# kluonj/HelFEM

Measured on AMD Instinct MI355X. Metric: scf_iteration_wall_time_fock_plus_geneig_nbf4230, lower is better.
Workload: dtype f64; 1 GPU; diatomic Z1=7 Z2=7 R=2.068 PBE, nelem=5 nnodes=15 nquad=75 lmmax=[20,20] (Nbf=4230, Nang=61, Nrad=70), XC grid 92x13, symmetry blocks [1380, 1470, 1380]: J+XC Fock build + eig_gsym_sub + density per step; parallelism=shard1, density=occupied orbitals of the core Hamiltonian

## Files before the change

### helfem_amd/csrc/hip/capi.cpp

```cpp
#include "internal.h"
#include "../host/checkpoint.h"
#include "../host/diis.h"
#include "../host/dftfuncs.h"
#include <cstring>
#include <memory>
#include <mutex>

namespace hfg {
static thread_local std::string g_err;
void set_error(const std::string &msg) { g_err = msg; }

}

using namespace hfg;

#define HFG_TRY try {
#define HFG_CATCH                       \
  }                                     \
  catch (const std::logic_error &e) {   \
    hfg::set_error(e.what());           \
    return 1;                           \
  }                                     \
  catch (const std::runtime_error &e) { \
    hfg::set_error(e.what());           \
// ... 664 lines not shown
  if (nP == 0) return false;
  if (!in || !out) throw std::logic_error(std::string(who) + ": null matrix pointer\n");
  return true;
}
int hfg_coulomb_batch_devptr(hfg_ctx *ctx, hfg_basis *b, int64_t nP, const double *dP, double *dJ) {
  HFG_TRY
  if (coulomb_batch_args("hfg_coulomb_batch_devptr", ctx, b, nP, dP, dJ)) coulomb_batch_dev(ctx, b, nP, dP, dJ);
  HFG_CATCH
}
int hfg_exchange_dev(hfg_ctx *ctx, hfg_basis *b, const double *dP, double *dK) {
  HFG_TRY exchange_dev(ctx, b, dP, dK);
  HFG_CATCH
}
int hfg_exchange_occ_dev(hfg_ctx *ctx, hfg_basis *b, const double *dP, const double *dC, int64_t nocc, double *dK) {
  HFG_TRY
  if (nocc < 1 || !dC) throw std::logic_error("hfg_exchange_occ_dev: occupied orbitals missing\n");
  exchange_dev(ctx, b, dP, dK, false, dC, (int)nocc);
  HFG_CATCH
}
int hfg_rs_exchange_dev(hfg_ctx *ctx, hfg_basis *b, const double *dP, double *dK) {
  HFG_TRY exchange_dev(ctx, b, dP, dK, true);
  HFG_CATCH
}
int hfg_xc_fock_dev(hfg_ctx *ctx, hfg_basis *b, int x_func, int c_func, const double *dP, double *dH, double *dScal,
                    double thr) {
  HFG_TRY xc_fock_dev(ctx, b, x_func, c_func, dP, dH, dScal, thr);
  HFG_CATCH
}
int hfg_xc_fock_pol_dev(hfg_ctx *ctx, hfg_basis *b, int x_func, int c_func, const double *dPa, const double *dPb,
                        double *dHa, double *dHb, double *dScal, double thr) {
  HFG_TRY xc_fock_pol_dev(ctx, b, x_func, c_func, dPa, dPb, dHa, dHb, dScal, thr);
  HFG_CATCH
}
int hfg_eig_gsym_sub_dev(hfg_ctx *ctx, int64_t N, const double *dF, const double *dS, int nblk, const int64_t *blk_ptr,
                         const int64_t *blk_idx, double *dE, double *dC) {
  HFG_TRY eig_gsym_sub_dev(ctx, (int)N, dF, dS, nblk, blk_ptr, blk_idx, dE, dC);
  HFG_CATCH
}
int64_t hfg_eig_block_buf_size(int nblk, const int64_t *blk_ptr) { return (int64_t)eig_block_buf_size(nblk, blk_ptr); }
int hfg_eig_blocks_dev(hfg_ctx *ctx, int64_t N, const double *dF, const double *dS, int nblk, const int64_t *blk_ptr,
                       const int64_t *blk_idx, double *dBlockBuf) {
  HFG_TRY eig_blocks_dev(ctx, (int)N, dF, dS, nblk, blk_ptr, blk_idx, dBlockBuf);
  HFG_CATCH
}
int hfg_eig_assemble_dev(hfg_ctx *ctx, int64_t N, int nblk, const int64_t *blk_ptr, const int64_t *blk_idx,
                         const double *dBlockBuf, double *dE, double *dC) {
  HFG_TRY eig_assemble_dev(ctx, (int)N, nblk, blk_ptr, blk_idx, dBlockBuf, dE, dC);
  HFG_CATCH
}
int hfg_form_density_dev(hfg_ctx *ctx, int64_t N, int64_t ncols, const double *dC, int64_t nocc, double *dP) {
  HFG_TRY form_density_dev(ctx, (int)N, (int)ncols, dC, (int)nocc, dP);
  HFG_CATCH
}
int hfg_gemm_dev(hfg_ctx *ctx, int tA, int tB, int64_t m, int64_t n, int64_t k, const double *dA, int64_t lda,
                 const double *dB, int64_t ldb, double *dC, int64_t ldc) {
  HFG_TRY gemm_dev(ctx, tA != 0, tB != 0, (int)m, (int)n, (int)k, 1.0, dA, (int)lda, dB, (int)ldb, 0.0, dC, (int)ldc);
  HFG_CATCH
}

int64_t hfg_fock_compact_size(hfg_basis *b) { return (int64_t)fock_compact_size(b); }
int hfg_fock_compact_dev(hfg_ctx *ctx, hfg_basis *b, int x_func, int c_func, const double *dP, double *dFc,
                         double *dScal, double thr) {
  HFG_TRY fock_compact_dev(ctx, b, x_func, c_func, dP, dFc, dScal, thr);
  HFG_CATCH
}
int hfg_fock_finish_dev(hfg_ctx *ctx, hfg_basis *b, const double *dFc, const double *dH0, const int *dBlockId,
// ... 410 lines not shown
```

### helfem_amd/csrc/hip/fock.hip

```cpp
#include "internal.h"
#include "xc_device.h"
#include "../host/dftfuncs.h"
#include <cstring>

namespace hfg {

__global__ void k_gather_compact(const double *__restrict__ P, int N, int A, int R, int E, int p,
                                 const int *__restrict__ shell_off, const int *__restrict__ shell_skip,
                                 double *__restrict__ Xc) {
  int blk = blockIdx.x;
  int e = blk % E;
  int xy = blk / E;
  int y = xy % A, x = xy / A;
  int pp = p * p;
  for (int t = threadIdx.x; t < pp; t += blockDim.x) {
    int i = t % p, j = t / p;
    int ni = e * (p - 1) + i, nj = e * (p - 1) + j;
    double v = 0.0;
    bool ok = (ni < R) && (nj < R) && !(shell_skip[x] && ni == 0) && !(shell_skip[y] && nj == 0);
    if (ok) v = P[(size_t)(shell_off[y] + nj) * N + (shell_off[x] + ni)];
    Xc[(size_t)blk * pp + t] = v;
  }
}

// ... 524 lines not shown
          s0 += sB[i * nq + q] * pv;
          s1 += sdB[i * nq + q] * pv;
        }
        d0 += s0 * sB[j * nq + q];
        d1 += s1 * sB[j * nq + q];
        d2 += s1 * sdB[j * nq + q];
        if (do_lapl) d3 += s0 * sL[j * nq + q];
      }
    if (q < nq && jc < NJ) {
      part[(0 * NJ + jc) * nq + q] = d0;
      part[(1 * NJ + jc) * nq + q] = d1;
      part[(2 * NJ + jc) * nq + q] = d2;
      if (do_lapl) part[(3 * NJ + jc) * nq + q] = d3;
    }
    __syncthreads();
    if (jc == 0 && q < nq && (e * nq + q) % nranks == rank) {
      double a0 = 0.0, a1 = 0.0, a2 = 0.0, a3 = 0.0;
      for (int k = 0; k < NJ; k++) {
        a0 += part[(0 * NJ + k) * nq + q];
        a1 += part[(1 * NJ + k) * nq + q];
        a2 += part[(2 * NJ + k) * nq + q];
        if (do_lapl) a3 += part[(3 * NJ + k) * nq + q];
      }
      const size_t Q = (size_t)e * nq + q;
      D0[Q * AA + xy] = a0;
      if (do_grad) D1[Q * AA + xy] = a1;
      if (do_tau) D2[Q * AA + xy] = a2;
      if (do_lapl) D3[Q * AA + xy] = a3;
    }
    __syncthreads();
  }
}

__global__ void k_xc_density_theta(const double *__restrict__ D0, const double *__restrict__ D1,
                                   const double *__restrict__ D2, const double *__restrict__ D3, const double *__restrict__ Th,
                                   const double *__restrict__ dTh, const int *__restrict__ shell_l,
                                   const double *__restrict__ rad_sh, int A, int nth, int G,
                                   const int *__restrict__ grp_off, const int *__restrict__ grp_shell, int do_grad,
                                   int do_tau, int do_lapl, size_t NQ, int rank, int nranks, double *__restrict__ V) {
  extern __shared__ double sh[];
  size_t Q = blockIdx.x;
  if ((int)(Q % nranks) != rank) return;
  int ga = blockIdx.y / G, gb = blockIdx.y % G;
  int a0 = grp_off[ga], na = grp_off[ga + 1] - a0;
  int b0 = grp_off[gb], nb = grp_off[gb + 1] - b0;
  double *d0 = sh, *d1 = sh + na * nb, *d2 = sh + 2 * na * nb, *d3 = sh + 3 * na * nb;
  size_t AA = (size_t)A * A;
  const double ir2 = do_lapl ? 1.0 / (rad_sh[Q] * rad_sh[Q]) : 0.0;
  for (int t = threadIdx.x; t < na * nb; t += blockDim.x) {
    int ia = t / nb, ib = t % nb;
    int a = grp_shell[a0 + ia], b = grp_shell[b0 + ib];
    d0[t] = D0[Q * AA + (size_t)a * A + b];
    d1[t] = do_grad ? D1[Q * AA + (size_t)a * A + b] : 0.0;
    d2[t] = do_tau ? D2[Q * AA + (size_t)a * A + b] : 0.0;
    if (do_lapl) d3[t] = D3[Q * AA + (size_t)a * A + b] - (double)(shell_l[b] * (shell_l[b] + 1)) * ir2 * d0[t];
  }
  __syncthreads();
  for (int i = threadIdx.x; i < nth; i += blockDim.x) {
    double r = 0.0, s = 0.0, u = 0.0, k3 = 0.0, k4 = 0.0, k5 = 0.0;
    for (int ia = 0; ia < na; ia++) {
      int a = grp_shell[a0 + ia];
      double s0 = 0.0, s1 = 0.0, s2 = 0.0, s3 = 0.0, s5 = 0.0;
      for (int ib = 0; ib < nb; ib++) {
        double tb = Th[(size_t)grp_shell[b0 + ib] * nth + i];
        s0 += d0[ia * nb + ib] * tb;
        s1 += d1[ia * nb + ib] * tb;
// ... 915 lines not shown
  XCPlan pl;
  pl.do_grad = either(xc::is_gga);
  pl.do_lapl = either(xc::is_mgga_lapl);
  if (pl.do_lapl && t->geom != 1) throw std::logic_error("Laplacian not implemented!\n");
  pl.do_tau = either(xc::is_mgga) || pl.do_lapl;
  pl.ext = either(xc::is_ext);
  pl.thr = pl.do_tau ? std::max(thr, 1e-40) : thr;
  pl.maxgrp = 0;
  for (int g = 0; g < t->G; g++) pl.maxgrp = std::max(pl.maxgrp, t->h_grp_off[g + 1] - t->h_grp_off[g]);
  pl.NQ = (size_t)t->E * t->nq;
  pl.AA = (size_t)t->A * t->A;
  pl.nv = pl.NQ * t->G * t->G * t->ntheta;
  return pl;
}

static void xc_buffers(FockAux &a, const XCPlan &pl, int planes) {
  a.D0.resize(pl.NQ * pl.AA);
  a.D1.resize(pl.NQ * pl.AA);
  a.GA.resize(pl.NQ * pl.AA);
  a.GB.resize(pl.NQ * pl.AA);
  if (pl.do_tau) {
    a.D2.resize(pl.NQ * pl.AA);
    a.GC.resize(pl.NQ * pl.AA);
  }
  if (pl.do_lapl) {
    a.D3.resize(pl.NQ * pl.AA);
    a.GL.resize(pl.NQ * pl.AA);
  }
  a.V.resize(planes * pl.nv);
  a.Fo.resize(planes * pl.nv);
  a.partial.resize(3 * pl.NQ);
}

static void xc_density_stage(hfg_ctx *ctx, const hfg_dev_tables *t, FockAux &a, const XCPlan &pl, const double *dPc, double *dV) {
  const int A = t->A, E = t->E, p = t->p, nq = t->nq, G = t->G, nth = t->ntheta;
  hipLaunchKernelGGL(k_xc_density_radial, dim3(A * A, E), dim3(256), xc_density_radial_lds(p, nq, pl.do_lapl), ctx->stream, dPc,
                     t->rad_B.p, t->rad_dB.p, (const double *)t->rad_L.p, A, E, p, nq, pl.do_grad, pl.do_tau, pl.do_lapl,
                     ctx->shard_rank, ctx->shard_n, a.D0.p, a.D1.p, a.D2.p, a.D3.p);
  hipLaunchKernelGGL(k_xc_density_theta, dim3((unsigned)pl.NQ, G * G), dim3(std::min(256, round_up64(nth))),
                     (pl.do_lapl ? 4 : 3) * pl.maxgrp * pl.maxgrp * sizeof(double), ctx->stream, a.D0.p, a.D1.p, (const double *)a.D2.p,
                     (const double *)a.D3.p, t->Th.p, t->dTh.p, t->shell_l.p, t->rad_sh.p, A, nth, G, t->grp_off.p, t->grp_shell.p,
                     pl.do_grad, pl.do_tau, pl.do_lapl, pl.NQ, ctx->shard_rank, ctx->shard_n, dV);
}

static void xc_fock_stage(hfg_ctx *ctx, const hfg_dev_tables *t, FockAux &a, const XCPlan &pl, double *dFo, double *dHc) {
  const int A = t->A, E = t->E, p = t->p, nq = t->nq;
  launch_xc_fock_theta(ctx, pl.NQ, t->G, t->ntheta, pl.maxgrp, dFo, t->Th.p, t->dTh.p, A, t->grp_off.p, t->grp_shell.p, pl.do_grad,
                       pl.do_tau, ctx->shard_rank, ctx->shard_n, a.GA.p, a.GB.p, a.GC.p, pl.do_lapl, a.GL.p);
  hipLaunchKernelGGL(k_xc_fock_radial, dim3(A * A, E), dim3(std::min(256, round_up64(p * p))), xc_fock_radial_lds(p, nq, pl.do_lapl),
                     ctx->stream, a.GA.p, a.GB.p, (const double *)a.GC.p, (const double *)a.GL.p, t->rad_B.p, t->rad_dB.p,
                     (const double *)t->rad_L.p, t->shell_l.p, t->rad_sh.p, A, E, p, nq, pl.do_grad, pl.do_tau, pl.do_lapl, ctx->shard_rank,
                     ctx->shard_n, dHc);
}

template <typename K, typename... Tail>
static void launch_xc_grid(hfg_ctx *ctx, const hfg_dev_tables *t, FockAux &a, const XCPlan &pl, K k_ext, K k_plain, size_t shb,
                           int x_func, int c_func, Tail... tail) {
  K k = pl.ext ? k_ext : k_plain;
  if (shb > 64 * 1024) HFG_HIP_CHECK(hipFuncSetAttribute((const void *)k, hipFuncAttributeMaxDynamicSharedMemorySize, (int)shb));
  hipLaunchKernelGGL(k, dim3((unsigned)pl.NQ), dim3(256), shb, ctx->stream, a.V.p, t->rad_w.p, t->rad_sh.p, t->th_s.p, t->th_w.p,
                     t->grp_m.p, t->cosd.p, t->sind.p, t->Dmax, t->G, t->ntheta, t->nphi, t->Rhalf, t->geom, x_func, c_func, pl.do_grad,
                     pl.do_tau, pl.do_lapl, pl.thr, pl.NQ, ctx->shard_rank, ctx->shard_n, a.Fo.p, a.partial.p, tail...);
}

static void xc_compact(hfg_ctx *ctx, hfg_basis *basis, int x_func, int c_func, const double *dPc, double *dHc, double *dScal,
                       double thr) {
  hfg_dev_tables *t = tables_of(ctx, basis);
  const XCPlan pl = xc_plan(t, x_func, c_func, thr);
  FockAux &a = aux_for(ctx, basis);
  const int npl = pl.do_lapl ? 6 : 5;
  xc_buffers(a, pl, npl);
// ... 72 lines not shown
      HFG_XC_EVAL_POINT_POL(true, id, ra, rb, saa, sab, sbb, ta, tb, la, lb, r0 >= thr, r1 >= thr, e, va, vb, vsaa, vsab, vsbb, vta, vtb, vla, vlb);
      if (!std::isfinite(vla)) vla = 0.0;
      if (!std::isfinite(vlb)) vlb = 0.0;
    }
    out(exc, i, e);
    out(vrho, 2 * i, va);
    out(vrho, 2 * i + 1, vb);
    out(vsigma, 3 * i, vsaa);
    out(vsigma, 3 * i + 1, vsab);
    out(vsigma, 3 * i + 2, vsbb);
    out(vlapl, 2 * i, vla);
    out(vlapl, 2 * i + 1, vlb);
    out(vtau, 2 * i, vta);
    out(vtau, 2 * i + 1, vtb);
  }
}

void xc_eval_host_ext(int id, const double *pars, int npars, int nspin, size_t np, const double *rho, const double *sigma,
                      const double *lapl, const double *tau, double *exc, double *vrho, double *vsigma, double *vlapl, double *vtau,
                      double thr) {
  if (npars > 0 && !pars) throw std::runtime_error("Functional parameters missing.\n");
  xc::XCPar par = HFG_XCPAR_DEFAULTS;
  if (npars > 0) {
    const helfem::XCFunc *f = helfem::find_xc_func(id);
    if (f && f->npar > 0 && !strcmp(f->role, "c")) helfem::check_xc_params(0, 0, id, npars);
    else helfem::check_xc_params(id, npars, 0, 0);
    fill_xcpar(par, id, pars, npars);
  }
  struct Reset {
    ~Reset() { xc::host_xcpar() = xc::XCPar HFG_XCPAR_DEFAULTS; }
  } reset;
  xc::host_xcpar() = par;
  xc_eval_host(id, nspin, np, rho, sigma, lapl, tau, exc, vrho, vsigma, vlapl, vtau, thr);
}

void xc_fock_dev(hfg_ctx *ctx, hfg_basis *basis, int x_func, int c_func, const double *dP, double *dH, double *dScal,
                 double thr) {
  hfg_dev_tables *t = tables_of(ctx, basis);
  FockAux &a = aux_for(ctx, basis);
  const size_t nc = (size_t)t->A * t->A * t->E * t->p * t->p;
  a.Pc.resize(nc);
  a.Jc.resize(nc);
  ProfScope ps(ctx, "xc");
  gather_compact(ctx, basis, dP, a.Pc.p);
  xc_compact(ctx, basis, x_func, c_func, a.Pc.p, a.Jc.p, dScal, thr);
  scatter_dense(ctx, basis, a.Jc.p, dH);
  HFG_HIP_CHECK(hipGetLastError());
}

static void xc_compact_pol(hfg_ctx *ctx, hfg_basis *basis, int x_func, int c_func, const double *dPca, const double *dPcb,
                           double *dHca, double *dHcb, double *dScal, double thr) {
  hfg_dev_tables *t = tables_of(ctx, basis);
  const XCPlan pl = xc_plan(t, x_func, c_func, thr);
  FockAux &a = aux_for(ctx, basis);
  const int npl = pl.do_lapl ? 6 : (pl.do_tau ? 5 : 3);
  xc_buffers(a, pl, 2 * npl);
  for (int sp = 0; sp < 2; sp++) xc_density_stage(ctx, t, a, pl, sp ? dPcb : dPca, a.V.p + (size_t)sp * npl * pl.nv);
  const int npot2 = pl.do_lapl ? 12 : (pl.do_tau ? 10 : 8);
  int rowc = t->ntheta;
  while ((size_t)(npot2 * rowc * t->nphi + 3 * 4) * sizeof(double) > tuning().xc_lds_limit && rowc > 1) rowc = (rowc + 1) / 2;
  size_t shb = (size_t)(npot2 * rowc * t->nphi + 3 * 4) * sizeof(double);
  if (shb > 150 * 1024) throw std::runtime_error("XC angular grid too large for the polarised grid kernel's LDS tile");
  launch_xc_grid(ctx, t, a, pl, k_xc_grid_pol<true>, k_xc_grid_pol<false>, shb, x_func, c_func, rowc);
  for (int sp = 0; sp < 2; sp++) xc_fock_stage(ctx, t, a, pl, a.Fo.p + (size_t)sp * npl * pl.nv, sp ? dHcb : dHca);
  hipLaunchKernelGGL(k_xc_sum_partials, dim3(1), dim3(64), 0, ctx->stream, a.partial.p, pl.NQ, dScal);
  HFG_HIP_CHECK(hipGetLastError());
// ... 112 lines not shown
```

### helfem_amd/csrc/hip/internal.h

```cpp
#pragma once
#include "common.h"
#include "tables.h"
#include "../host/scf.h"

namespace hfg {

enum class GemmTile { Auto, T64, T128, T128x64 };
struct GemmHow {
  GemmTile tile = GemmTile::Auto;
  bool acc = false, split2 = false, map = false;
};
void gemm_tasklist_dev(hfg_ctx *ctx, const GemmTask *dtasks, int ntasks, int maxM, int maxN, GemmHow how = {});
void gemm_worklist_dev(hfg_ctx *ctx, const GemmTask *dtasks, const int2 *dwl, int nwg, GemmTile tile, bool split2 = false);
void gemm_worklist(const std::vector<GemmTask> &tasks, GemmTile tile, bool split2, std::vector<int2> &out);
void gemm_mirror_lower_dev(hfg_ctx *ctx, const GemmTask *dtasks, int ntasks, int maxN);
bool gemm_prefers_128(hfg_ctx *ctx, long tiles128);
void gemm_dev(hfg_ctx *ctx, bool tA, bool tB, int M, int N, int K, double alpha, const double *A, int lda, const double *B, int ldb,
              double beta, double *C, int ldc);

void coulomb_dev(hfg_ctx *ctx, hfg_basis *basis, const double *dP, double *dJ);
void coulomb_batch_dev(hfg_ctx *ctx, hfg_basis *basis, int64_t nP, const double *dP, double *dJ);
void coulomb_energy_matrix_dev(hfg_ctx *ctx, hfg_basis *basis, int64_t nP, const double *dP, double *dW);
void set_xc_params(hfg_ctx *ctx, int x_func, const double *x_pars, int nx, int c_func, const double *c_pars, int nc);
void xc_eval_host(int id, int nspin, size_t np, const double *rho, const double *sigma, const double *lapl, const double *tau,
                  double *exc, double *vrho, double *vsigma, double *vlapl, double *vtau, double thr);
void xc_eval_host_ext(int id, const double *pars, int npars, int nspin, size_t np, const double *rho, const double *sigma,
                      const double *lapl, const double *tau, double *exc, double *vrho, double *vsigma, double *vlapl, double *vtau,
                      double thr);
void xc_fock_dev(hfg_ctx *ctx, hfg_basis *basis, int x_func, int c_func, const double *dP, double *dH, double *dScal,
                 double thr);
void xc_fock_pol_dev(hfg_ctx *ctx, hfg_basis *basis, int x_func, int c_func, const double *dPa, const double *dPb, double *dHa,
                     double *dHb, double *dScal, double thr);
void model_potential_dev(hfg_ctx *ctx, hfg_basis *basis, int kind1, int Z1, double d1, double H1, int kind2, int Z2, double d2,
                         double H2, double *dH);
size_t fock_compact_size(hfg_basis *basis);
void fock_compact_dev(hfg_ctx *ctx, hfg_basis *basis, int x_func, int c_func, const double *dP, double *dFc, double *dScal,
                      double thr);
void fock_finish_dev(hfg_ctx *ctx, hfg_basis *basis, const double *dFc, const double *dH0, const int *dBlockId,
                     double *dF);

void exchange_dev(hfg_ctx *ctx, hfg_basis *basis, const double *dP, double *dK, bool rs = false, const double *Lknown = nullptr,
                  int rknown = 0);
bool exchange_lowrank_dev(hfg_ctx *ctx, hfg_dev_tables *t, const double *dP, double *dK, const double *Lknown,
                          int rknown);

void compute_tei_dev(hfg_ctx *ctx, hfg_basis *basis);

void compute_rs_tei_dev(hfg_ctx *ctx, hfg_basis *basis, int rs_kind, double omega);
void rs_special_dev(hfg_ctx *ctx, int which, int L, const double *a, const double *b, size_t n, double *out);

void eig_sym_dev(hfg_ctx *ctx, int n, const double *dA, double *dE, double *dC);
void eig_gsym_dev(hfg_ctx *ctx, int N, int n, const double *dF, const double *dS, double *dE, double *dC);
void eig_gsym_sub_dev(hfg_ctx *ctx, int N, const double *dF, const double *dS, int nblk, const int64_t *blk_ptr,
                      const int64_t *blk_idx, double *dE, double *dC);
void eig_gsym_sub_pair_dev(hfg_ctx *ctx, int N, const double *dFa, const double *dFb, const double *dS, int nblk,
                           const int64_t *blk_ptr, const int64_t *blk_idx, double *dEa, double *dCa, double *dEb,
                           double *dCb);
size_t eig_block_buf_size(int nblk, const int64_t *blk_ptr);
void eig_blocks_dev(hfg_ctx *ctx, int N, const double *dF, const double *dS, int nblk, const int64_t *blk_ptr,
                    const int64_t *blk_idx, double *dBlockBuf);
void eig_assemble_dev(hfg_ctx *ctx, int N, int nblk, const int64_t *blk_ptr, const int64_t *blk_idx, const double *dBlockBuf,
                      double *dE, double *dC);
void eig_block_supports(hfg_ctx *ctx, int N, const double *dS, int nblk, const int64_t *blk_ptr, const int64_t *blk_idx,
                        std::vector<int64_t> &cols);
int64_t eig_sel_count(int nblk, const int64_t *blk_ptr, int64_t nev);
// ... 28 lines not shown
```

### helfem_amd/csrc/hip/tables.cpp

```cpp
#include "internal.h"
#include <algorithm>
#include <cmath>
#include <functional>
#include <set>

namespace hfg {


namespace {
struct BasisView {
  int geom = 0;
  int A = 0, R = 0, E = 0, p = 0, nq = 0, N = 0, Nd = 0;
  double Rhalf = 0.0;
  helfem::IVec lval, mval;
  std::vector<int> skip;
  std::vector<std::pair<int, int> > LM_map, lm_map;
  std::vector<int> lm_tab;
  std::vector<double> LM_fac;
  int Ntab = 0, ntt = 4, ndt = 4, Lp1 = 0;
  int rs_kind = 0, pair_tei = 0;
  std::function<const helfem::Mat &(int, int, int)> tei_pair;
  std::function<void(int, int, int &, int &)> Lrange;
  std::function<double(int, int, int)> c0, c2;
  std::function<const helfem::Mat &(int, int, int)> disj, tei;
// ... 347 lines not shown
                for (size_t rj = 0; rj < Ni; rj++)
                  for (size_t ri = 0; ri < Ni; ri++)
                    stage[((cj + lof) * p + (ci + lof)) * pp + (rj + lo) * p + (ri + lo)] = m(rj * Ni + ri, cj * Nf + ci);
            HFG_HIP_CHECK(hipMemcpyAsync(dst, stage.data(), blk * sizeof(double), hipMemcpyHostToDevice, s));
            HFG_HIP_CHECK(hipStreamSynchronize(s));
          }
        }
    HFG_HIP_CHECK(hipStreamSynchronize(s));
  }
  t->have_tei = true;

  if (ldft > 0 && mdft > 0) {
    const int nq = t->nq;
    t->ntheta = ldft;
    t->nphi = mdft;
    std::vector<double> B((size_t)E * nq * p, 0.0), dB((size_t)E * nq * p, 0.0), rw((size_t)E * nq), rsh((size_t)E * nq);
    for (int e = 0; e < E; e++) {
      helfem::Mat bf = b.bf(e), df = b.df(e);
      helfem::Vec w = b.wrad(e), r = b.rcoord(e);
      const int lo = b.lo(e);
      for (int q = 0; q < nq; q++) {
        for (size_t i = 0; i < bf.n_cols; i++) {
          B[((size_t)e * nq + q) * p + i + lo] = bf(q, i);
          dB[((size_t)e * nq + q) * p + i + lo] = df(q, i);
        }
        rw[(size_t)e * nq + q] = w[q];
        rsh[(size_t)e * nq + q] = r[q];
      }
    }
    t->rad_B.upload(B, s);
    t->rad_dB.upload(dB, s);
    t->rad_w.upload(rw, s);
    t->rad_sh.upload(rsh, s);
    if (b.lf) {
      std::vector<double> Lr((size_t)E * nq * p, 0.0);
      for (int e = 0; e < E; e++) {
        helfem::Mat df = b.df(e), lf = b.lf(e);
        helfem::Vec r = b.rcoord(e);
        const int lo = b.lo(e);
        for (int q = 0; q < nq; q++)
          for (size_t i = 0; i < lf.n_cols; i++) Lr[((size_t)e * nq + q) * p + i + lo] = lf(q, i) + 2.0 * df(q, i) / r[q];
      }
      t->rad_L.upload(Lr, s);
    }

    helfem::Vec xc, wc;
    helfem::chebyshev_rule(ldft, xc, wc);
    std::vector<double> ths(ldft), Th((size_t)A * ldft), dTh((size_t)A * ldft);
    for (int i = 0; i < ldft; i++) ths[i] = sqrt(1.0 - xc[i] * xc[i]);
    for (int a = 0; a < A; a++)
      for (int i = 0; i < ldft; i++) {
        Th[(size_t)a * ldft + i] = helfem::theta_lm(b.lval[a], b.mval[a], xc[i]);
        dTh[(size_t)a * ldft + i] = helfem::dtheta_lm(b.lval[a], b.mval[a], xc[i]);
      }
    t->th_c.upload(xc, s);
    t->th_s.upload(ths, s);
    t->th_w.upload(wc, s);
    t->Th.upload(Th, s);
    t->dTh.upload(dTh, s);

    std::set<int> mset(b.mval.begin(), b.mval.end());
    std::vector<int> gm(mset.begin(), mset.end());
    t->G = (int)gm.size();
    std::vector<int> goff(t->G + 1, 0), gshell, sgrp(A);
    for (int g = 0; g < t->G; g++) {
      goff[g] = (int)gshell.size();
// ... 30 lines not shown
```

### helfem_amd/csrc/hip/tables.h

```cpp
#pragma once
#include "common.h"

struct hfg_dev_tables {
  int A = 0, R = 0, E = 0, p = 0, nq = 0, N = 0, Nd = 0, NLM = 0, Nlm = 0;
  int T = 0;
  int geom = 0;
  int Ntab = 0;
  int ntt = 4;
  int ndt = 4;
  int dQ0 = 2;
  int Lp1 = 0;
  double Rhalf = 0.0;
  bool have_tei = false, have_xc = false;
  int rs_kind = 0;
  int pair_tei = 0;

  hfg::DevBuf<int> shell_l, shell_m, shell_off, shell_skip;
  hfg::DevBuf<int> pair_off, ent_iLM;
  hfg::DevBuf<double> ent_c0, ent_c2;
  hfg::DevBuf<int> lm_off, lm_x, lm_y;
  hfg::DevBuf<double> lm_c0, lm_c2;
  hfg::DevBuf<int> LM_ilm, LM_partner;
  hfg::DevBuf<int> lm_tab;
  hfg::DevBuf<int> LM_tab;
  hfg::DevBuf<double> LM_fac;
  hfg::DevBuf<double> disj, tei;

  int ntheta = 0, nphi = 0, G = 0;
  hfg::DevBuf<double> rad_B, rad_dB;
  hfg::DevBuf<double> rad_L;
  hfg::DevBuf<double> rad_w, rad_sh;
  hfg::DevBuf<double> th_c, th_s, th_w;
  hfg::DevBuf<double> Th, dTh;
  hfg::DevBuf<int> grp_m, grp_off, grp_shell;
  hfg::DevBuf<int> shell_grp;
  hfg::DevBuf<double> cosd, sind;
  int Dmax = 0;

  std::vector<int> h_LM_L, h_LM_M, h_LM_ilm, h_grp_off, h_shell_l, h_shell_m, h_shell_skip, h_lm_tab;
  std::vector<double> h_LM_fac;
  std::vector<double> h_c0tab, h_c2tab;

  hfg::WorkspaceOwner<hfg::WS_TABLE_SLOTS> work;
};

namespace hfg {
void upload_basis_tables(hfg_ctx *ctx, hfg_basis *basis, int ldft, int mdft, bool with_rs);
}
```

### helfem_amd/csrc/host/tuning.h

```cpp
#pragma once
#include <string>

namespace helfem {
constexpr int EXL_GMAX = 16;
enum class TrdMode { persistent, chain, twokernel, unblocked };
enum class EigSel { crossover, stein, dc };
enum class RsTei { host, dev };
#define HELFEM_TUNING(X) \
  X(scf_host, bool, false, "HELFEM_SCF", true, "=host", !strcmp(e, "host"), "SCF loop driven from the host through the per-stage entry points (checker of the device-resident loop)") \
  X(tei_host, bool, false, "HELFEM_TEI", false, "=host", !strcmp(e, "host"), "in-element tables built by the threaded host code and uploaded (checker of tei_dev.hip)") \
  X(rs_tei, RsTei, RsTei::host, "HELFEM_RS_TEI", false, "word", !strcmp(e, "dev") ? RsTei::dev : RsTei::host, "range-separated exchange tables of the SCF drivers: dev = built on the device (rs_tei_dev.hip); unset or any other word = built by the threaded host code and uploaded") \
  X(exchange_general, bool, false, "HELFEM_EXCHANGE", true, "=general", !strcmp(e, "general"), "general exchange kernels always, not only where the low-rank fast path declines") \
  X(exl_rb, int, 0, "HELFEM_EXL_RB", false, "int", atoi(e), "RB kernel of the low-rank exchange: 4 the 4 x 4 vector kernel, 1 the one-pair vector kernel (checkers), else the matrix-core kernel k_exl_RBm") \
  X(exl_mgroups, bool, true, "HELFEM_EXL_MGROUPS", false, "off if 0", atoi(e) != 0, "cross-element products by blocks of equal m; off: the full products") \
  X(exl_rect, int, -1, "HELFEM_EXL_RECT", false, "int", atoi(e), "tiles of the element GEMM: 0 / 1 / 2 = 128 x 128 / 128 x 64 / 64 x 64 always; negative: 64 x 64 when the tasks average fewer than 1500 pairs, else 128 x 128") \
  X(exl_wl, bool, true, "HELFEM_EXL_WL", false, "off if 0", atoi(e) != 0, "XCD-contiguous workgroup lists for the element GEMM and the cross products; off: plain task-list grids") \
  X(exl_splitk, bool, true, "HELFEM_EXL_SPLITK", false, "off if 0", atoi(e) != 0, "two half-K workgroups per tile for the cross products; off: one workgroup per tile") \
  X(exl_crect, bool, true, "HELFEM_EXL_CRECT", false, "off if 0", atoi(e) != 0, "128 x 64 tiles for the split cross products; off: 128 x 128") \
  X(exl_groups, int, 4, "HELFEM_EXL_GROUPS", false, "int", std::max(1, std::min(EXL_GMAX, atoi(e))), "groups of 64 factors tried before the general kernels take over, clamped to 1 ... 16") \
  X(exl_hint, bool, true, "HELFEM_EXL_HINT", false, "off if 0", atoi(e) != 0, "the SCF loop's occupied orbitals taken as the factors of P; off: always factorise and verify P (checker)") \
  X(exl_pair, bool, true, "HELFEM_EXL_PAIR", false, "off if 0", atoi(e) != 0, "low-rank fast path for the pair (erfc) tables; off: general kernels") \
  X(fock_overlap, bool, true, "HELFEM_FOCK_OVERLAP", false, "off if 0", atoi(e) != 0, "Coulomb kernels on the side stream beside the XC kernels; off: one after the other on the main stream") \
  X(xc_lds_limit, size_t, 150 * 1024, "HELFEM_XC_LDS_LIMIT", false, "int", (size_t)atol(e), "bytes of LDS the angular XC kernels plan with; smaller forces the chunked kernels (tests)") \
  X(coulomb_batch_chunk, int, 0, "HELFEM_COULOMB_BATCH_CHUNK", true, "int", std::max(0, atoi(e)), "densities per pass over the tables of the batched Coulomb build forced smaller than the LDS rule allows (tests; 0: the rule's own)") \
  X(diis_blocks, bool, true, "HELFEM_DIIS_BLOCKS", false, "off if 0", atoi(e) != 0, "DIIS error per symmetry block; off: the four dense N^3 products (checker)") \
  X(diis_lowrank, bool, true, "HELFEM_DIIS_LOWRANK", false, "off if 0", atoi(e) != 0, "blocked DIIS error from the occupied orbitals; off: per-block n^3 products from F and P (checker)") \
  X(eig_pair, bool, true, "HELFEM_EIG_PAIR", false, "off if 0", atoi(e) != 0, "both spins' Fock matrices in one batched eigensolve; off: two calls") \
  X(trd_mode, TrdMode, TrdMode::persistent, "HELFEM_TRD", false, "word", !strcmp(e, "persistent") ? TrdMode::persistent : !strcmp(e, "twokernel") ? TrdMode::twokernel : !strcmp(e, "unblocked") ? TrdMode::unblocked : TrdMode::chain, "tridiagonalisation: persistent = k_trdp where the batch fits, else the chain; chain (and any unknown word) = one k_trdf launch per column always (checker); twokernel = k_trdb_gemv + k_trdb_w; unblocked = the first-generation kernels") \
  X(trdp_min, int, 256, "HELFEM_TRDP_MIN", false, "int", atoi(e), "smallest order the persistent kernel takes") \
  X(trdp_r, int, 0, "HELFEM_TRDP_R", false, "int", atoi(e), "rows per thread of the persistent kernel forced (0: the first that fits)") \
  X(trdp_u, int, 0, "HELFEM_TRDP_U", false, "int", atoi(e), "column chunks per thread of the persistent kernel forced wider than needed (measurement; 0: narrowest)") \
  X(trdp_limit_ms, long long, 200, "HELFEM_TRDP_LIMIT_MS", false, "int", atoll(e), "wall-clock bound of every spin of the persistent kernel, ms") \
  X(trdp_phases, bool, true, "HELFEM_TRDP_PHASES", false, "off if 0", atoi(e) != 0, "one cooperative launch per phase; off: the whole matrix in one launch (checker)") \
  X(trdp_step, int, 96, "HELFEM_TRDP_STEP", false, "int", std::max(1, atoi(e)), "fewest columns of a phase (at least 1)") \
  X(trdp_coop, bool, true, "HELFEM_TRDP_COOP", false, "off if 0", atoi(e) != 0, "hipLaunchCooperativeKernel for the phases; off: plain launches (A/B of the launch overhead)") \
  X(trdp_stamps, int, 0, "HELFEM_TRDP_STAMPS", false, "int", atoi(e), "non-zero: the stamping kernels, one launch per eigensolve, phase summary on stderr; 2 and more: also per-column stamps of one workgroup") \
  X(trdp_stamps_file, std::string, "", "HELFEM_TRDP_STAMPS_FILE", false, "path", e, "with stamps: file for the stamps of every workgroup over 64 columns (tools/trdp_window.py)") \
  X(trd_tail, int, 2, "HELFEM_TRD_TAIL", false, "int", atoi(e), "last columns of the chain in one launch: 0 none, 1 the LDS-resident kernel (order 128), else the register-resident kernel (order 192)") \
  X(trdf_sym, int, -1, "HELFEM_TRDF_SYM", false, "int", atoi(e), "symmetric sweep of k_trdf: 0 never, other non-negative always, negative by HELFEM_TRDF_SYM_MIN") \
  X(trdf_sym_min, int, 0, "HELFEM_TRDF_SYM_MIN", false, "int", atoi(e), "panels whose full grid has more tiles than this sweep one triangle only") \
  X(trd_band_update, bool, true, "HELFEM_TRD_BAND_UPDATE", false, "off if 0", atoi(e) != 0, "band-limited trailing updates when every sweep is symmetric; off: full updates") \
  X(trdf_nth, int, 0, "HELFEM_TRDF_NTH", false, "int", atoi(e), "512: k_trdf with 512 threads; anything else 1024 (A/B runs)") \
  X(acc_tile, int, 0, "HELFEM_ACC_TILE", false, "int", atoi(e), "128: 128 x 128 tiles for the accumulating updates (and full, not band-limited ones); anything else 64 x 64") \
  X(trdf_dbg, int, 0, "HELFEM_TRDF_DBG", false, "int", atoi(e), "measurement replay of k_trdf only: bits 0-2 go to the kernel's debug field, bit 2 also prints the per-wave stamps (tools/trdf_probe.py)") \
  X(trdf_c, int, -1, "HELFEM_TRDF_C", false, "int", atoi(e), "measurement replay of k_trdf only: column-in-panel index forced for every launch (negative: each launch's own)") \
  X(tridiag_ql, bool, false, "HELFEM_TRIDIAG", false, "=ql", !strcmp(e, "ql"), "one-lane implicit QL for the tridiagonal problem instead of divide and conquer (checker)") \
  X(dc_gemm_small, bool, false, "HELFEM_DC_GEMM", false, "=small", !strcmp(e, "small"), "Q U of the divide-and-conquer merges by the first 64 x 64 kernel instead of the tile engine (checker)") \
  X(dc_levels, bool, false, "HELFEM_DC", false, "=levels", !strcmp(e, "levels"), "divide-and-conquer merges with the gather, scatter and copy-back passes over Q and ten launches per level (checker of the column-mapped product)") \
  X(eigsel, EigSel, EigSel::crossover, "HELFEM_EIGSEL", false, "word", !strcmp(e, "stein") ? EigSel::stein : !strcmp(e, "dc") ? EigSel::dc : EigSel::crossover, "selected eigenpairs (hfg_eig_*_sel): stein = multisection and inverse iteration always; dc = the full divide and conquer, then the lowest columns (checker); unset or any other word = the crossover, which sends every wanted fraction to dc (measured: stein is slower down to 1/64 of the columns)") \
  X(dc_dbg, bool, false, "HELFEM_DC_DBG", false, "present", true, "merge statistics of divide and conquer on stderr") \
  X(bt_column, bool, false, "HELFEM_BT", false, "=column", !strcmp(e, "column"), "back-transformation reflector by reflector instead of compact WY (checker)") \
  X(bt_fold, bool, true, "HELFEM_BT_FOLD", false, "off if 0", atoi(e) != 0, "X Q formed on the side stream beside divide and conquer; off: Z <- Q Z on the main stream behind it") \
  X(bt_side, bool, false, "HELFEM_BT_SIDE", false, "=1", atoi(e) == 1, "without the fold: the compact-WY set-up on the side stream") \
  X(gemm_tile, int, 0, "HELFEM_GEMM_TILE", false, "int", atoi(e), "128: 128 x 128 tiles always; other non-zero: 64 x 64 always; 0: the large tiles where they fill whole rounds of the chip") \
  X(gemm_splitk, int, -1, "HELFEM_GEMM_SPLITK", false, "int", atoi(e), "eigensolve's products: 0 / other non-negative = large tiles without / with two half-K workgroups each; negative: chosen by tile count") \
// ... 15 lines not shown
```

### include/helfem_gpu.h

```cpp
#ifndef HELFEM_GPU_H
#define HELFEM_GPU_H

#include <stddef.h>
#include <stdint.h>

#ifdef __cplusplus
extern "C" {
#endif

typedef struct hfg_ctx hfg_ctx;
typedef struct hfg_basis hfg_basis;

#define HFG_NULL_STREAM ((void *)(intptr_t)-1)
int hfg_ctx_create(hfg_ctx **ctx, int device, void *stream);
int hfg_ctx_destroy(hfg_ctx *ctx);
int hfg_ctx_synchronize(hfg_ctx *ctx);
const char *hfg_last_error(void);
const char *hfg_version(void);
int hfg_device_count(void);

int hfg_ctx_set_shard(hfg_ctx *ctx, int rank, int nranks);

int hfg_ctx_fix_sinvh(hfg_ctx *ctx, const double *dSinvh);

// ... 101 lines not shown
int hfg_basis_radial_table(const hfg_basis *basis, int which, int iel, double *out, int64_t *rows, int64_t *cols);
typedef struct {
  int kind;
  int Z;
  double d, H;
} hfg_model_pot;
int hfg_model_potential(hfg_ctx *ctx, hfg_basis *basis, const hfg_model_pot *p1, const hfg_model_pot *p2, double *H);
int hfg_scf_set_iguess(int iguess);
int hfg_eig_gsym(hfg_ctx *ctx, int64_t N, int64_t n, const double *F, const double *Sinvh, double *E, double *C);
int hfg_eig_gsym_sub(hfg_ctx *ctx, int64_t N, const double *F, const double *Sinvh, int nblk,
                     const int64_t *blk_ptr, const int64_t *blk_idx, double *E, double *C);
int hfg_eig_gsym_sub_pair(hfg_ctx *ctx, int64_t N, const double *Fa, const double *Fb, const double *Sinvh, int nblk,
                          const int64_t *blk_ptr, const int64_t *blk_idx, double *Ea, double *Ca, double *Eb, double *Cb);
int hfg_eig_sym(hfg_ctx *ctx, int64_t n, const double *A, double *E, double *C);
int64_t hfg_eig_sel_count(int nblk, const int64_t *blk_ptr, int64_t nev);
int hfg_eig_sym_sel(hfg_ctx *ctx, int64_t n, const double *A, int64_t nev, double *E, double *C);
int hfg_eig_gsym_sub_sel(hfg_ctx *ctx, int64_t N, const double *F, const double *Sinvh, int nblk, const int64_t *blk_ptr,
                         const int64_t *blk_idx, int64_t nev, double *E , double *C );
int hfg_form_sinvh(hfg_ctx *ctx, int64_t N, const double *S, int chol, int nblk, const int64_t *blk_ptr,
                   const int64_t *blk_idx, double *Sinvh);
int hfg_form_density(hfg_ctx *ctx, int64_t N, int64_t ncols, const double *C, int64_t nocc, double *P);
int hfg_gemm(hfg_ctx *ctx, int transA, int transB, int64_t m, int64_t n, int64_t k, const double *A, int64_t lda,
             const double *B, int64_t ldb, double *C, int64_t ldc);

int hfg_coulomb_dev(hfg_ctx *ctx, hfg_basis *basis, const double *dP, double *dJ);
int hfg_coulomb_batch_devptr(hfg_ctx *ctx, hfg_basis *basis, int64_t nP, const double *dP, double *dJ);
int hfg_exchange_dev(hfg_ctx *ctx, hfg_basis *basis, const double *dP, double *dK);
int hfg_rs_exchange_dev(hfg_ctx *ctx, hfg_basis *basis, const double *dP, double *dK);
int hfg_exchange_occ_dev(hfg_ctx *ctx, hfg_basis *basis, const double *dP, const double *dC, int64_t nocc, double *dK);
int hfg_xc_fock_dev(hfg_ctx *ctx, hfg_basis *basis, int x_func, int c_func, const double *dP, double *dH,
                    double *dScal, double dens_thr);
int hfg_xc_fock_pol_dev(hfg_ctx *ctx, hfg_basis *basis, int x_func, int c_func, const double *dPa, const double *dPb,
                        double *dHa, double *dHb, double *dScal , double dens_thr);
int64_t hfg_fock_compact_size(hfg_basis *basis);
int hfg_fock_compact_dev(hfg_ctx *ctx, hfg_basis *basis, int x_func, int c_func, const double *dP, double *dFc,
                         double *dScal, double dens_thr);
int hfg_fock_finish_dev(hfg_ctx *ctx, hfg_basis *basis, const double *dFc, const double *dH0, const int *dBlockId,
                        double *dF);
int hfg_eig_gsym_sub_dev(hfg_ctx *ctx, int64_t N, const double *dF, const double *dSinvh, int nblk,
                         const int64_t *blk_ptr, const int64_t *blk_idx, double *dE, double *dC);
int hfg_eig_gsym_sub_sel_dev(hfg_ctx *ctx, int64_t N, const double *dF, const double *dSinvh, int nblk, const int64_t *blk_ptr,
                             const int64_t *blk_idx, int64_t nev, double *dE , double *dC );
int64_t hfg_eig_block_buf_size(int nblk, const int64_t *blk_ptr);
int hfg_eig_blocks_dev(hfg_ctx *ctx, int64_t N, const double *dF, const double *dSinvh, int nblk,
                       const int64_t *blk_ptr, const int64_t *blk_idx, double *dBlockBuf);
int hfg_eig_assemble_dev(hfg_ctx *ctx, int64_t N, int nblk, const int64_t *blk_ptr, const int64_t *blk_idx,
                         const double *dBlockBuf, double *dE, double *dC);
int hfg_form_density_dev(hfg_ctx *ctx, int64_t N, int64_t ncols, const double *dC, int64_t nocc, double *dP);
int hfg_gemm_dev(hfg_ctx *ctx, int transA, int transB, int64_t m, int64_t n, int64_t k, const double *dA,
                 int64_t lda, const double *dB, int64_t ldb, double *dC, int64_t ldc);

int hfg_scf_diatomic(hfg_ctx *ctx, int Z1, int Z2, double Rbond, const int *lmmax, int nlm, int nelem, int nnodes,
                     int nquad, double Rmax, int igrid, double zexp, int lpad, const char *method, int ldft, int mdft,
                     int symmetry, int multiplicity, int maxit, double convthr, int verbose, double *out );

#define HFG_MAX_LMMAX 16
typedef struct hfg_scf_options {
  int program;
  int Z1, Z2;
  double Rbond;
  int nela, nelb, Q, M;
  int lmmax[HFG_MAX_LMMAX];
  int nlm;
  int lmax, mmax;
  int lpad;
  double Rmax;
// ... 104 lines not shown
```

Measured before the change: 8.467 ms.

## Add register-tiled ordered and MFMA radial XC density kernels

Replaces the default radial density contraction (one workgroup per shell pair) with an ordered kernel where each wave handles four shell pairs, lanes map to quadrature points, and the B/dB tables sit in LDS. The goal is to reuse the basis tables across pairs and cut launch granularity while matching the scalar kernel bit for bit. An optional MFMA kernel, enabled by a tuning flag, contracts against precomputed product tables uploaded at setup and rounds differently. Debug entry points are also added to compare the radial densities.

Result: no change. 8.467 ms (+0.0%).

```diff
diff --git a/helfem_amd/csrc/hip/capi.cpp b/helfem_amd/csrc/hip/capi.cpp
--- a/helfem_amd/csrc/hip/capi.cpp
+++ b/helfem_amd/csrc/hip/capi.cpp
@@ -720,6 +720,14 @@
   HFG_TRY xc_fock_pol_dev(ctx, b, x_func, c_func, dPa, dPb, dHa, dHb, dScal, thr);
   HFG_CATCH
 }
+int hfg_debug_xc_radial_density(hfg_ctx *ctx, hfg_basis *b, int planes, const double *dPc, double *dD) {
+  HFG_TRY xc_radial_density_debug(ctx, b, planes, dPc, dD);
+  HFG_CATCH
+}
+int hfg_debug_xc_radial_tables(hfg_ctx *ctx, hfg_basis *b, double *hB, double *hdB) {
+  HFG_TRY xc_radial_tables_debug(ctx, b, hB, hdB);
+  HFG_CATCH
+}
 int hfg_eig_gsym_sub_dev(hfg_ctx *ctx, int64_t N, const double *dF, const double *dS, int nblk, const int64_t *blk_ptr,
                          const int64_t *blk_idx, double *dE, double *dC) {
   HFG_TRY eig_gsym_sub_dev(ctx, (int)N, dF, dS, nblk, blk_ptr, blk_idx, dE, dC);
diff --git a/helfem_amd/csrc/hip/fock.hip b/helfem_amd/csrc/hip/fock.hip
--- a/helfem_amd/csrc/hip/fock.hip
+++ b/helfem_amd/csrc/hip/fock.hip
@@ -580,6 +580,146 @@
   }
 }
 
+constexpr int XO_XT = 4;
+__global__ __launch_bounds__(256) void k_xc_density_radial_ord(const double *__restrict__ Pc, const double *__restrict__ B,
+                                                               const double *__restrict__ dB, int AA, int E, int p, int nq, int NJ,
+                                                               int do_grad, int do_tau, int rank, int nranks, double *__restrict__ D0,
+                                                               double *__restrict__ D1, double *__restrict__ D2) {
+  extern __shared__ double sh[];
+  const int e = blockIdx.y, pp = p * p;
+  double *sB = sh, *sdB = sh + p * nq;
+  for (int t = threadIdx.x; t < p * nq; t += blockDim.x) {
+    int q = t / p, i = t % p;
+    sB[i * nq + q] = B[((size_t)e * nq + q) * p + i];
+    sdB[i * nq + q] = dB[((size_t)e * nq + q) * p + i];
+  }
+  __syncthreads();
+  const int wave = __builtin_amdgcn_readfirstlane((int)(threadIdx.x >> 6)), lane = threadIdx.x & 63;
+  const int xy0 = (blockIdx.x * 4 + wave) * XO_XT;
+  if (xy0 >= AA) return;
+  const double *Px[XO_XT];
+#pragma unroll
+  for (int x = 0; x < XO_XT; x++) Px[x] = Pc + ((size_t)min(xy0 + x, AA - 1) * E + e) * pp;
+  for (int q0 = 0; q0 < nq; q0 += 64) {
+    const int q = q0 + lane, qc = min(q, nq - 1);
+    double a0[XO_XT], a1[XO_XT], a2[XO_XT];
+#pragma unroll
+    for (int x = 0; x < XO_XT; x++) a0[x] = a1[x] = a2[x] = 0.0;
+    for (int jc = 0; jc < NJ; jc++) {
+      double d0[XO_XT], d1[XO_XT], d2[XO_XT];
+#pragma unroll
+      for (int x = 0; x < XO_XT; x++) d0[x] = d1[x] = d2[x] = 0.0;
+      for (int j = jc; j < p; j += NJ) {
+        double s0[XO_XT], s1[XO_XT];
+#pragma unroll
+        for (int x = 0; x < XO_XT; x++) s0[x] = s1[x] = 0.0;
+        for (int i = 0; i < p; i++) {
+          const double b = sB[i * nq + qc], db = sdB[i * nq + qc];
+#pragma unroll
+          for (int x = 0; x < XO_XT; x++) {
+            const double pv = Px[x][j * p + i];
+            s0[x] = fma(b, pv, s0[x]);
+            s1[x] = fma(db, pv, s1[x]);
+          }
+        }
+        const double bj = sB[j * nq + qc], dbj = sdB[j * nq + qc];
+#pragma unroll
+        for (int x = 0; x < XO_XT; x++) {
+          d0[x] = fma(s0[x], bj, d0[x]);
+          d1[x] = fma(s1[x], bj, d1[x]);
+          d2[x] = fma(s1[x], dbj, d2[x]);
+        }
+      }
+#pragma unroll
+      for (int x = 0; x < XO_XT; x++) {
+        a0[x] += d0[x];
+        a1[x] += d1[x];
+        a2[x] += d2[x];
+      }
+    }
+    const size_t Q = (size_t)e * nq + qc;
+    if (q < nq && (int)(Q % nranks) == rank) {
+#pragma unroll
+      for (int x = 0; x < XO_XT; x++)
+        if (xy0 + x < AA) {
+          D0[Q * AA + xy0 + x] = a0[x];
+          if (do_grad) D1[Q * AA + xy0 + x] = a1[x];
+          if (do_tau) D2[Q * AA + xy0 + x] = a2[x];
+        }
+    }
+  }
+}
+
+constexpr int XR_XT = 64, XR_KC = 16, XR_QG = 5;
+template <int NPL>
+__global__ __launch_bounds__(256) void k_xc_density_radial_mfma(const double *__restrict__ Pc, const double *__restrict__ Wk, int AA, int E,
+                                                                int pp, int nq, int KP, int QP, int do_grad, int rank, int nranks,
+                                                                double *__restrict__ D0, double *__restrict__ D1,
+                                                                double *__restrict__ D2) {
+  __shared__ double sW[NPL][XR_KC][16 * XR_QG];
+  __shared__ double sP[XR_XT][XR_KC + 2];
+  const int xy0 = blockIdx.x * XR_XT, e = blockIdx.y, q0 = blockIdx.z * 16 * XR_QG;
+  const int ncg = min(16 * XR_QG, QP - q0) / 16;
+  const int nqt = min(XR_QG, (nq - q0 + 15) / 16);
+  const int lane = threadIdx.x & 63, wave = threadIdx.x >> 6, l15 = lane & 15, l4 = lane >> 4;
+  const int lr = threadIdx.x >> 4, lc = threadIdx.x & 15;
+  const double *Wb = Wk + (size_t)e * 3 * KP * QP + q0;
+  cb_d4 acc[NPL][XR_QG];
+#pragma unroll
+  for (int pl = 0; pl < NPL; pl++)
+#pragma unroll
+    for (int qt = 0; qt < XR_QG; qt++) acc[pl][qt] = cb_d4{0.0, 0.0, 0.0, 0.0};
+  double rw[NPL][XR_QG], rp[XR_XT / 16];
+  auto load = [&](int c0) {
+#pragma unroll
+    for (int pl = 0; pl < NPL; pl++)
+#pragma unroll
+      for (int u = 0; u < XR_QG; u++) rw[pl][u] = (u < ncg) ? Wb[((size_t)pl * KP + c0 + lr) * QP + lc + 16 * u] : 0.0;
+#pragma unroll
+    for (int u = 0; u < XR_XT / 16; u++) {
+      const int xy = xy0 + lr + 16 * u, k = c0 + lc;
+      rp[u] = (xy < AA && k < pp) ? Pc[((size_t)xy * E + e) * pp + k] : 0.0;
+    }
+  };
+  load(0);
+  for (int c0 = 0; c0 < KP; c0 += XR_KC) {
+    __syncthreads();
+#pragma unroll
+    for (int pl = 0; pl < NPL; pl++)
+#pragma unroll
+      for (int u = 0; u < XR_QG; u++) sW[pl][lr][lc + 16 * u] = rw[pl][u];
+#pragma unroll
+    for (int u = 0; u < XR_XT / 16; u++) sP[lr + 16 * u][lc] = rp[u];
+    __syncthreads();
+    if (c0 + XR_KC < KP) load(c0 + XR_KC);
+#pragma unroll
+    for (int k0 = 0; k0 < XR_KC; k0 += 4) {
+      const double b = sP[16 * wave + l15][k0 + l4];
+#pragma unroll
+      for (int qt = 0; qt < XR_QG; qt++)
+        if (qt < nqt) {
+#pragma unroll
+          for (int pl = 0; pl < NPL; pl++)
+            acc[pl][qt] = __builtin_amdgcn_mfma_f64_16x16x4f64(sW[pl][k0 + l4][16 * qt + l15], b, acc[pl][qt], 0, 0, 0);
+        }
+    }
+  }
+  const int xy = xy0 + 16 * wave + l15;
+  if (xy >= AA) return;
+#pragma unroll
+  for (int qt = 0; qt < XR_QG; qt++)
+#pragma unroll
+    for (int r = 0; r < 4; r++) {
+      const int q = q0 + 16 * qt + l4 + 4 * r;
+      if (qt >= nqt || q >= nq) continue;
+      const size_t Q = (size_t)e * nq + q;
+      if ((int)(Q % nranks) != rank) continue;
+      D0[Q * AA + xy] = acc[0][qt][r];
+      if (NPL > 1 && do_grad) D1[Q * AA + xy] = acc[NPL > 1 ? 1 : 0][qt][r];
+      if (NPL > 2) D2[Q * AA + xy] = acc[NPL > 2 ? 2 : 0][qt][r];
+    }
+}
+
 __global__ void k_xc_density_theta(const double *__restrict__ D0, const double *__restrict__ D1,
                                    const double *__restrict__ D2, const double *__restrict__ D3, const double *__restrict__ Th,
                                    const double *__restrict__ dTh, const int *__restrict__ shell_l,
@@ -1561,11 +1701,30 @@
   a.partial.resize(3 * pl.NQ);
 }
 
-static void xc_density_stage(hfg_ctx *ctx, const hfg_dev_tables *t, FockAux &a, const XCPlan &pl, const double *dPc, double *dV) {
-  const int A = t->A, E = t->E, p = t->p, nq = t->nq, G = t->G, nth = t->ntheta;
+static void launch_xc_density_radial(hfg_ctx *ctx, const hfg_dev_tables *t, const XCPlan &pl, const double *dPc, double *D0, double *D1,
+                                     double *D2, double *D3) {
+  const int A = t->A, E = t->E, p = t->p, nq = t->nq;
+  if (!pl.do_lapl && tuning().xc_radial == 0 && 2 * (size_t)p * nq * sizeof(double) <= 64 * 1024) {
+    const int NJ = 256 / nq > 0 ? std::min(256 / nq, p) : 1;
+    hipLaunchKernelGGL(k_xc_density_radial_ord, dim3((A * A + 4 * XO_XT - 1) / (4 * XO_XT), E), dim3(256),
+                       2 * (size_t)p * nq * sizeof(double), ctx->stream, dPc, (const double *)t->rad_B.p, (const double *)t->rad_dB.p,
+                       A * A, E, p, nq, NJ, pl.do_grad, pl.do_tau, ctx->shard_rank, ctx->shard_n, D0, D1, D2);
+    return;
+  }
+  if (!pl.do_lapl && tuning().xc_radial == 2) {
+    const dim3 grid((A * A + XR_XT - 1) / XR_XT, E, (nq + 16 * XR_QG - 1) / (16 * XR_QG));
+    auto k = pl.do_tau ? k_xc_density_radial_mfma<3> : pl.do_grad ? k_xc_density_radial_mfma<2> : k_xc_density_radial_mfma<1>;
+    hipLaunchKernelGGL(k, grid, dim3(256), 0, ctx->stream, dPc, (const double *)t->rad_Wk.p, A * A, E, p * p, nq, t->xw_kp, t->xw_qp,
+                       pl.do_grad, ctx->shard_rank, ctx->shard_n, D0, D1, D2);
+    return;
+  }
   hipLaunchKernelGGL(k_xc_density_radial, dim3(A * A, E), dim3(256), xc_density_radial_lds(p, nq, pl.do_lapl), ctx->stream, dPc,
                      t->rad_B.p, t->rad_dB.p, (const double *)t->rad_L.p, A, E, p, nq, pl.do_grad, pl.do_tau, pl.do_lapl,
-                     ctx->shard_rank, ctx->shard_n, a.D0.p, a.D1.p, a.D2.p, a.D3.p);
+                     ctx->shard_rank, ctx->shard_n, D0, D1, D2, D3);
+}
+static void xc_density_stage(hfg_ctx *ctx, const hfg_dev_tables *t, FockAux &a, const XCPlan &pl, const double *dPc, double *dV) {
+  const int A = t->A, G = t->G, nth = t->ntheta;
+  launch_xc_density_radial(ctx, t, pl, dPc, a.D0.p, a.D1.p, a.D2.p, a.D3.p);
   hipLaunchKernelGGL(k_xc_density_theta, dim3((unsigned)pl.NQ, G * G), dim3(std::min(256, round_up64(nth))),
                      (pl.do_lapl ? 4 : 3) * pl.maxgrp * pl.maxgrp * sizeof(double), ctx->stream, a.D0.p, a.D1.p, (const double *)a.D2.p,
                      (const double *)a.D3.p, t->Th.p, t->dTh.p, t->shell_l.p, t->rad_sh.p, A, nth, G, t->grp_off.p, t->grp_shell.p,
@@ -1704,6 +1863,32 @@
   } reset;
   xc::host_xcpar() = par;
   xc_eval_host(id, nspin, np, rho, sigma, lapl, tau, exc, vrho, vsigma, vlapl, vtau, thr);
+}
+
+static XCPlan xc_radial_debug_plan(const hfg_dev_tables *t, int planes) {
+  if (!t->have_xc) throw std::runtime_error("XC grid tables were not uploaded (hfg_basis_upload with ldft,mdft > 0)\n");
+  if (planes < 1 || planes > 3) throw std::logic_error("hfg_debug_xc_radial_*: planes must be 1, 2 or 3\n");
+  XCPlan pl{};
+  pl.do_grad = planes >= 2;
+  pl.do_tau = planes >= 3;
+  pl.NQ = (size_t)t->E * t->nq;
+  pl.AA = (size_t)t->A * t->A;
+  return pl;
+}
+void xc_radial_density_debug(hfg_ctx *ctx, hfg_basis *basis, int planes, const double *dPc, double *dD) {
+  hfg_dev_tables *t = tables_of(ctx, basis);
+  const XCPlan pl = xc_radial_debug_plan(t, planes);
+  const size_t n = pl.NQ * pl.AA;
+  launch_xc_density_radial(ctx, t, pl, dPc, dD, dD + (planes > 1 ? n : 0), dD + (planes > 2 ? 2 * n : 0), nullptr);
+  HFG_HIP_CHECK(hipGetLastError());
+}
+void xc_radial_tables_debug(hfg_ctx *ctx, hfg_basis *basis, double *hB, double *hdB) {
+  hfg_dev_tables *t = tables_of(ctx, basis);
+  if (!t->have_xc) throw std::runtime_error("XC grid tables were not uploaded (hfg_basis_upload with ldft,mdft > 0)\n");
+  const size_t nb = (size_t)t->E * t->nq * t->p * sizeof(double);
+  HFG_HIP_CHECK(hipMemcpyAsync(hB, t->rad_B.p, nb, hipMemcpyDeviceToHost, ctx->stream));
+  HFG_HIP_CHECK(hipMemcpyAsync(hdB, t->rad_dB.p, nb, hipMemcpyDeviceToHost, ctx->stream));
+  HFG_HIP_CHECK(hipStreamSynchronize(ctx->stream));
 }
 
 void xc_fock_dev(hfg_ctx *ctx, hfg_basis *basis, int x_func, int c_func, const double *dP, double *dH, double *dScal,
diff --git a/helfem_amd/csrc/hip/internal.h b/helfem_amd/csrc/hip/internal.h
--- a/helfem_amd/csrc/hip/internal.h
+++ b/helfem_amd/csrc/hip/internal.h
@@ -31,6 +31,8 @@
                  double thr);
 void xc_fock_pol_dev(hfg_ctx *ctx, hfg_basis *basis, int x_func, int c_func, const double *dPa, const double *dPb, double *dHa,
                      double *dHb, double *dScal, double thr);
+void xc_radial_density_debug(hfg_ctx *ctx, hfg_basis *basis, int planes, const double *dPc, double *dD);
+void xc_radial_tables_debug(hfg_ctx *ctx, hfg_basis *basis, double *hB, double *hdB);
 void model_potential_dev(hfg_ctx *ctx, hfg_basis *basis, int kind1, int Z1, double d1, double H1, int kind2, int Z2, double d2,
                          double H2, double *dH);
 size_t fock_compact_size(hfg_basis *basis);
diff --git a/helfem_amd/csrc/hip/tables.cpp b/helfem_amd/csrc/hip/tables.cpp
--- a/helfem_amd/csrc/hip/tables.cpp
+++ b/helfem_amd/csrc/hip/tables.cpp
@@ -403,6 +403,22 @@
     t->rad_dB.upload(dB, s);
     t->rad_w.upload(rw, s);
     t->rad_sh.upload(rsh, s);
+    {
+      const int pp = p * p;
+      t->xw_kp = (pp + 15) / 16 * 16;
+      t->xw_qp = xw_pad16(nq);
+      std::vector<double> Wk((size_t)E * 3 * t->xw_kp * t->xw_qp, 0.0);
+      for (int e = 0; e < E; e++)
+        for (int q = 0; q < nq; q++) {
+          const double *Bq = &B[((size_t)e * nq + q) * p], *dBq = &dB[((size_t)e * nq + q) * p];
+          for (int j = 0; j < p; j++)
+            for (int i = 0; i < p; i++) {
+              const double w[3] = {Bq[i] * Bq[j], dBq[i] * Bq[j], dBq[i] * dBq[j]};
+              for (int pl = 0; pl < 3; pl++) Wk[(((size_t)e * 3 + pl) * t->xw_kp + j * p + i) * t->xw_qp + q] = w[pl];
+            }
+        }
+      t->rad_Wk.upload(Wk, s);
+    }
     if (b.lf) {
       std::vector<double> Lr((size_t)E * nq * p, 0.0);
       for (int e = 0; e < E; e++) {
diff --git a/helfem_amd/csrc/hip/tables.h b/helfem_amd/csrc/hip/tables.h
--- a/helfem_amd/csrc/hip/tables.h
+++ b/helfem_amd/csrc/hip/tables.h
@@ -29,6 +29,8 @@
   int ntheta = 0, nphi = 0, G = 0;
   hfg::DevBuf<double> rad_B, rad_dB;
   hfg::DevBuf<double> rad_L;
+  hfg::DevBuf<double> rad_Wk;
+  int xw_kp = 0, xw_qp = 0;
   hfg::DevBuf<double> rad_w, rad_sh;
   hfg::DevBuf<double> th_c, th_s, th_w;
   hfg::DevBuf<double> Th, dTh;
@@ -45,5 +47,6 @@
 };
 
 namespace hfg {
+inline int xw_pad16(int n) { return 16 * (((n + 15) / 16) | 1); }
 void upload_basis_tables(hfg_ctx *ctx, hfg_basis *basis, int ldft, int mdft, bool with_rs);
 }
diff --git a/helfem_amd/csrc/host/tuning.h b/helfem_amd/csrc/host/tuning.h
--- a/helfem_amd/csrc/host/tuning.h
+++ b/helfem_amd/csrc/host/tuning.h
@@ -21,6 +21,7 @@
   X(exl_hint, bool, true, "HELFEM_EXL_HINT", false, "off if 0", atoi(e) != 0, "the SCF loop's occupied orbitals taken as the factors of P; off: always factorise and verify P (checker)") \
   X(exl_pair, bool, true, "HELFEM_EXL_PAIR", false, "off if 0", atoi(e) != 0, "low-rank fast path for the pair (erfc) tables; off: general kernels") \
   X(fock_overlap, bool, true, "HELFEM_FOCK_OVERLAP", false, "off if 0", atoi(e) != 0, "Coulomb kernels on the side stream beside the XC kernels; off: one after the other on the main stream") \
+  X(xc_radial, int, 0, "HELFEM_XC_RADIAL", false, "word", !strcmp(e, "scalar") ? 1 : !strcmp(e, "mfma") ? 2 : 0, "radial density contraction X1 of the XC build: scalar (1) = one workgroup per shell pair (checker); mfma (2) = the matrix-core kernel on the product tables, which rounds differently; unset or any other word (0) = the ordered kernel, bitwise the scalar kernel's results (Laplacian plans always run the scalar kernel)") \
   X(xc_lds_limit, size_t, 150 * 1024, "HELFEM_XC_LDS_LIMIT", false, "int", (size_t)atol(e), "bytes of LDS the angular XC kernels plan with; smaller forces the chunked kernels (tests)") \
   X(coulomb_batch_chunk, int, 0, "HELFEM_COULOMB_BATCH_CHUNK", true, "int", std::max(0, atoi(e)), "densities per pass over the tables of the batched Coulomb build forced smaller than the LDS rule allows (tests; 0: the rule's own)") \
   X(diis_blocks, bool, true, "HELFEM_DIIS_BLOCKS", false, "off if 0", atoi(e) != 0, "DIIS error per symmetry block; off: the four dense N^3 products (checker)") \
diff --git a/include/helfem_gpu.h b/include/helfem_gpu.h
--- a/include/helfem_gpu.h
+++ b/include/helfem_gpu.h
@@ -157,6 +157,8 @@
                     double *dScal, double dens_thr);
 int hfg_xc_fock_pol_dev(hfg_ctx *ctx, hfg_basis *basis, int x_func, int c_func, const double *dPa, const double *dPb,
                         double *dHa, double *dHb, double *dScal , double dens_thr);
+int hfg_debug_xc_radial_density(hfg_ctx *ctx, hfg_basis *basis, int planes, const double *dPc, double *dD);
+int hfg_debug_xc_radial_tables(hfg_ctx *ctx, hfg_basis *basis, double *hB, double *hdB);
 int64_t hfg_fock_compact_size(hfg_basis *basis);
 int hfg_fock_compact_dev(hfg_ctx *ctx, hfg_basis *basis, int x_func, int c_func, const double *dP, double *dFc,
                          double *dScal, double dens_thr);
```
